# pettni/smooth_feedback

Hardware: AMD Instinct MI355X
Metric: QP solves/sec (higher is better)
Workload: dtype f64

## Files before the change

### smooth_feedback_amd/csrc/qp_sparse.hip

```cpp
#include <hip/hip_runtime.h>

#include <cstdlib>
#include <map>
#include <mutex>

#include <algorithm>
#include <type_traits>
#include <utility>
#include <cfloat>
#include <cmath>

#include "knobs.h"
#include "../../include/sfb.h"
#include "qp_sparse_kernel.h"
#include "wave_util.h"

#ifndef SFB_SWEEP_ASM
#define SFB_SWEEP_ASM 1
#endif
#ifndef SFB_SWEEP_DEPTH
#define SFB_SWEEP_DEPTH 8
#endif

namespace sfb {
// ... 990 lines not shown
                                              vdouble2 (&lx)[8], vint2 (&ix)[8], const bool pre, const bool next, const bool resident = false,
                                              const int treg = 0, const unsigned long long tail_have = 0)
{
  const int k = uni(pl.k);
  const int fu = uni(pl.funits) - treg;
  if (resident) sweep_dev<8, true, false, false, true, kLatResident>(pl.fidx, fu, w.LxF, t, lane, pl.fmask, 0, 0, lx, ix, pl.bidx, w.LxB, pl.bmask);
  else if (pre) sweep_dev<8, true, false, true, true>(pl.fidx, fu, w.LxF, t, lane, pl.fmask, 0, 0, lx, ix, pl.bidx, w.LxB, pl.bmask);
  else sweep_dev<8, true, false, false, true>(pl.fidx, fu, w.LxF, t, lane, pl.fmask, 0, 0, lx, ix, pl.bidx, w.LxB, pl.bmask);
  if constexpr (kLatTail > 0) {
    if (treg > 0) {
      double *const tl = t + (k - 1 - kLatTail) + lane;
      const bool mine = lane >= kLatTail - treg && lane <= kLatTail;
      double tr = mine ? *tl : 0.0;
      auto for_steps = [&]<int... S>(std::integer_sequence<int, S...>, auto &&fn) { (fn(std::integral_constant<int, S>{}), ...); };
      auto block = [&]<int B>(std::integral_constant<int, B>) {
        if (8 * B + 8 > kLatTail - treg) {
          for_steps(std::make_integer_sequence<int, 8>{}, [&]<int E>(std::integral_constant<int, E>) {
            constexpr int S = 8 * B + E;
            int l0, h0;
            asm volatile("v_accvgpr_read_b32 %0, a[%2] ; lat tail (check_sweep_spills.py)\n\tv_accvgpr_read_b32 %1, a[%3]"
                         : "=v"(l0), "=v"(h0)
                         : "n"(kLatTailReg0 + 2 * S), "n"(kLatTailReg0 + 2 * S + 1));
            const double piv = __hiloint2double(__builtin_amdgcn_readlane(__double2hiint(tr), S), __builtin_amdgcn_readlane(__double2loint(tr), S));
            if ((tail_have >> S) & 1) tr = fma(-__hiloint2double(h0, l0), piv, tr);
          });
        }
      };
      for_steps(std::make_integer_sequence<int, kLatTail / 8>{}, block);
      if (mine && lane > kLatTail - treg) *tl = tr;
      wave_lds_fence();
    }
  }
  for (int j0 = lane; j0 < k; j0 += kWave * 8) {
    double dv[8];
#pragma unroll
    for (int e = 0; e < 8; ++e) dv[e] = (j0 + e * kWave < k) ? Dinv[j0 + e * kWave] : 0.0;
#pragma unroll
    for (int e = 0; e < 8; ++e)
      if (j0 + e * kWave < k) t[j0 + e * kWave] = dv[e] * t[j0 + e * kWave];
  }
  wave_lds_fence();
  if (next) sweep_dev<8, true, false, true, true>(pl.bidx, uni(pl.bunits), w.LxB, t, lane, pl.bmask, 0, 0, lx, ix, pl.fidx, w.LxF, pl.fmask);
  else sweep_dev<8, true, false, true, false>(pl.bidx, uni(pl.bunits), w.LxB, t, lane, pl.bmask, 0, 0, lx, ix);
}

template<int UB>
__device__ __forceinline__ double lane_max_abs_b(const double *v, const int len, const int lane)
{
  double r = 0.0;
  for (int e0 = lane; e0 < len; e0 += kWave * UB) {
    double x[UB];
#pragma unroll
    for (int e = 0; e < UB; ++e) x[e] = (e0 + e * kWave < len) ? v[e0 + e * kWave] : 0.0;
#pragma unroll
    for (int e = 0; e < UB; ++e) r = fmax(r, fabs(x[e]));
  }
  return wave_max(r);
}
__device__ __forceinline__ double lane_max_abs(const double *v, int len, int lane)
{
  double r = 0.0;
  for (int e = lane; e < len; e += kWave) r = fmax(r, fabs(v[e]));
  return wave_max(r);
}

constexpr int kRowChunk = 8;
template<class PosF, class IdxF>
__device__ __forceinline__ double sp_row_dot(const int p0, const int p1, const double *vals, PosF pos, IdxF idx,
                                             const double *v)
{
  double s = 0.0;
  for (int q = p0; q < p1; q += kRowChunk) {
    int ps[kRowChunk], ix[kRowChunk];
    double a[kRowChunk], x[kRowChunk];
#pragma unroll
    for (int e = 0; e < kRowChunk; ++e) {
      const bool on = q + e < p1;
      ps[e] = on ? pos(q + e) : 0;
      ix[e] = on ? idx(q + e) : 0;
    }
#pragma unroll
    for (int e = 0; e < kRowChunk; ++e) {
      a[e] = vals[ps[e]];
      x[e] = v[ix[e]];
    }
#pragma unroll
    for (int e = 0; e < kRowChunk; ++e)
      if (q + e < p1) s = fma(a[e], x[e], s);
  }
  return s;
}
template<int RB, int CE, class PtrF, class PosF, class IdxF>
__device__ __forceinline__ void sp_rows_dot(double (&s)[RB], const int i0, const int nrows, PtrF ptr, const double *vals, PosF pos,
                                            IdxF idx, const double *v)
{
  int p[RB], pe[RB];
#pragma unroll
  for (int r = 0; r < RB; ++r) {
    const int i = i0 + r * kWave;
    const bool on = i < nrows;
    p[r]  = on ? ptr(i) : 0;
    pe[r] = on ? ptr(i + 1) : 0;
    s[r]  = 0.0;
  }
  for (;;) {
    bool more = false;
#pragma unroll
    for (int r = 0; r < RB; ++r) more = more || p[r] < pe[r];
    if (!more) break;
    int ps[RB][CE], ix[RB][CE];
    double a[RB][CE], x[RB][CE];
#pragma unroll
    for (int r = 0; r < RB; ++r)
#pragma unroll
      for (int e = 0; e < CE; ++e) {
        const bool on = p[r] + e < pe[r];
        ps[r][e] = on ? pos(p[r] + e) : 0;
        ix[r][e] = on ? idx(p[r] + e) : 0;
      }
#pragma unroll
    for (int r = 0; r < RB; ++r)
#pragma unroll
      for (int e = 0; e < CE; ++e) {
        a[r][e] = vals[ps[r][e]];
        x[r][e] = v[ix[r][e]];
      }
#pragma unroll
    for (int r = 0; r < RB; ++r) {
#pragma unroll
      for (int e = 0; e < CE; ++e)
        if (p[r] + e < pe[r]) s[r] = fma(a[r][e], x[r][e], s[r]);
      p[r] += CE;
    }
  }
}
template<int RB, int CE>
__device__ __forceinline__ void sp_rows_A(double (&s)[RB], const SparsePlanDev &pl, const Item &it, int i0, const double *v)
{
  sp_rows_dot<RB, CE>(s, i0, uni(pl.m), [&](int i) { return pl.Ap[i]; }, it.Ax, [](int p) { return p; },
                      [&](int p) { return pl.Aj[p]; }, v);
}
template<int RB, int CE>
__device__ __forceinline__ void sp_rows_P(double (&s)[RB], const SparsePlanDev &pl, const Item &it, int i0, const double *v)
{
  sp_rows_dot<RB, CE>(s, i0, uni(pl.n), [&](int i) { return pl.Prp[i]; }, it.Px, [&](int p) { return pl.Prpos[p]; },
                      [&](int p) { return pl.Prj[p]; }, v);
}
template<int RB, int CE>
__device__ __forceinline__ void sp_rows_At(double (&s)[RB], const SparsePlanDev &pl, const Item &it, int j0, const double *v)
{
  sp_rows_dot<RB, CE>(s, j0, uni(pl.n), [&](int j) { return pl.Acp[j]; }, it.Ax, [&](int p) { return pl.Acpos[p]; },
                      [&](int p) { return pl.Aci[p]; }, v);
}
__device__ __forceinline__ double sp_row_A(const SparsePlanDev &pl, const Item &it, int i, const double *v)
{
  return sp_row_dot(pl.Ap[i], pl.Ap[i + 1], it.Ax, [](int p) { return p; }, [&](int p) { return pl.Aj[p]; }, v);
}
__device__ __forceinline__ double sp_row_At(const SparsePlanDev &pl, const Item &it, int j, const double *v)
{
  return sp_row_dot(pl.Acp[j], pl.Acp[j + 1], it.Ax, [&](int p) { return pl.Acpos[p]; },
                    [&](int p) { return pl.Aci[p]; }, v);
}
__device__ __forceinline__ double sp_row_P(const SparsePlanDev &pl, const Item &it, int i, const double *v)
{
  return sp_row_dot(pl.Prp[i], pl.Prp[i + 1], it.Px, [&](int p) { return pl.Prpos[p]; },
                    [&](int p) { return pl.Prj[p]; }, v);
}

#ifdef SFB_CHECK_FULL_PASSES
constexpr bool kCheckExit = false;
#else
constexpr bool kCheckExit = true;
#endif
#ifdef SFB_PROF_CHECK
enum { kCkChecks, kCkOptimal, kCkDualRes, kCkOrdered, kCkPass2, kCkPinf, kCkPass3, kCkQdx, kCkRows, kCkDinf, kCkCycOpt, kCkCycCert, kCkCycPass2,
       kCkCycPass3, kCkCycTail, kCkHist2 = 16, kCkHist3 = 32, kCkSlots = 48 };
__device__ unsigned long long sfb_check_prof[2][kCkSlots];
constexpr int kStdWavesPerSimd = 2;
#define SFB_CK_ADD(slot, v) { if (lane == 0) atomicAdd(&sfb_check_prof[RBX > 4][slot], (unsigned long long)(v)); }
#define SFB_CK_LAP(slot) { const unsigned now_ = (unsigned)__builtin_amdgcn_s_memtime(); SFB_CK_ADD(slot, now_ - ck_pc) ck_pc = now_; }
#define SFB_CK_ROW(found, hit, base, j0) { if (!found && wave_ballot(hit)) { found = true; SFB_CK_ADD(base + min((j0) / kWave, 14), 1) } }
#define SFB_CK_HIST(base, found) { if (!found) SFB_CK_ADD(base + 15, 1) }
#else
constexpr int kStdWavesPerSimd = 3;
#define SFB_CK_ADD(slot, v)
#define SFB_CK_LAP(slot)
#define SFB_CK_ROW(found, hit, base, j0)
#define SFB_CK_HIST(base, found)
#endif

template<int RBX = 4>
__device__ inline int sp_check_stopping(const SparsePlanDev &pl, const Item &it, const Ws &w,
                                        const DenseKernelParams &kp, double *t, const int lane, float *score = nullptr)
{
  const int n = uni(pl.n), m = uni(pl.m);
  const double inf = INFINITY;
#ifdef SFB_PROF_CHECK
  unsigned ck_pc = (unsigned)__builtin_amdgcn_s_memtime();
  bool ck_first2 = false, ck_first3 = false;
#endif
  SFB_CK_ADD(kCkChecks, 1)
  const int chunk  = (uni(pl.k) + 1) / 2;
  const double *const xl = t, *const yl = t + n;
  {
    double a = 0.0, r = 0.0, z = 0.0;
    constexpr int RB = RBX, CE = 2;
    for (int i0 = lane; i0 < m; i0 += kWave * RB) {
      double Ax[RB], zi[RB];
#pragma unroll
      for (int rr = 0; rr < RB; ++rr) zi[rr] = (i0 + rr * kWave < m) ? w.zus[i0 + rr * kWave] : 0.0;
      sp_rows_A<RB, CE>(Ax, pl, it, i0, xl);
#pragma unroll
      for (int rr = 0; rr < RB; ++rr) {
        a = fmax(a, fabs(Ax[rr]));
        r = fmax(r, fabs(Ax[rr] - zi[rr]));
        z = fmax(z, fabs(zi[rr]));
      }
    }
    const double Ax_norm = wave_max(a), r_norm = wave_max(r), z_norm = wave_max(z);
    if (score != nullptr && lane == 0) *score = (float)(r_norm / (kp.eps_abs + kp.eps_rel * fmax(Ax_norm, z_norm)));
    if (r_norm <= kp.eps_abs + kp.eps_rel * fmax(Ax_norm, z_norm)) {
      SFB_CK_ADD(kCkDualRes, 1)
      double pn = 0.0, qn = 0.0, an = 0.0, rn = 0.0;
      if constexpr (RBX <= 4) {
      for (int j = lane; j < n; j += kWave) {
        const double Px = sp_row_P(pl, it, j, xl), Aty = sp_row_At(pl, it, j, yl), qj = it.q[j];
        pn = fmax(pn, fabs(Px));
        qn = fmax(qn, fabs(qj));
        an = fmax(an, fabs(Aty));
        rn = fmax(rn, fabs(Px + (qj + Aty)));
      }
      } else
      for (int j0 = lane; j0 < n; j0 += kWave * RB) {
        double Px[RB], Aty[RB], qj[RB];
#pragma unroll
        for (int rr = 0; rr < RB; ++rr) qj[rr] = (j0 + rr * kWave < n) ? it.q[j0 + rr * kWave] : 0.0;
        sp_rows_P<RB, CE>(Px, pl, it, j0, xl);
        sp_rows_At<RB, CE>(Aty, pl, it, j0, yl);
#pragma unroll
        for (int rr = 0; rr < RB; ++rr) {
          pn = fmax(pn, fabs(Px[rr]));
          qn = fmax(qn, fabs(qj[rr]));
          an = fmax(an, fabs(Aty[rr]));
          rn = fmax(rn, fabs(Px[rr] + (qj[rr] + Aty[rr])));
        }
      }
      const double dual_scale = fmax(fmax(wave_max(pn), wave_max(qn)), wave_max(an)), rn_norm = wave_max(rn);
      if (rn_norm <= kp.eps_abs + kp.eps_rel * dual_scale) {
        SFB_CK_ADD(kCkOptimal, 1)
        SFB_CK_LAP(kCkCycOpt)
        return SFB_QP_OPTIMAL;
      }
      if (score != nullptr && lane == 0) *score = (float)(rn_norm / (kp.eps_abs + kp.eps_rel * dual_scale));
    }
  }
  SFB_CK_LAP(kCkCycOpt)
  {
    constexpr int UBV     = RBX > 4 ? 6 : 1;
    const double Edy_norm = lane_max_abs_b<UBV>(w.dyus, m, lane);
    const double thr      = kp.eps_pinf * Edy_norm;
    int side = 2;
    {
      double ps = 0.0, pa = 0.0;
      bool brk0 = false;
      for (int i0 = lane; i0 < m; i0 += kWave * UBV) {
        double uv[UBV], lv[UBV], dv[UBV];
#pragma unroll
        for (int e = 0; e < UBV; ++e) {
          const int i   = i0 + e * kWave;
          const bool on = i < m;
          uv[e] = on ? it.u[i] : 0.0;
          lv[e] = on ? it.l[i] : 0.0;
          dv[e] = on ? w.dyus[i] : 0.0;
        }
#pragma unroll
        for (int e = 0; e < UBV; ++e) {
          if (i0 + e * kWave < m) {
            const double ui = uv[e], li = lv[e], dyi = dv[e];
            const double ta = (ui != inf) ? ui * fmax(0.0, dyi) : 0.0, tb = (li != -inf) ? li * fmin(0.0, dyi) : 0.0;
            ps += ta;
            ps += tb;
            pa += fabs(ta);
            pa += fabs(tb);
            brk0 = brk0 || (ui == inf && dyi > thr) || (li == -inf && dyi < -thr);
          }
        }
      }
      const double sum = wave_sum(ps), S = wave_sum(pa);
      const double err = 4.0 * (2.0 * (double)m) * DBL_EPSILON * S;
      if (!wave_ballot(brk0) && S < inf) {
        if (sum - err >= thr) side = 0;
        else if (sum + err < thr) side = 1;
      }
    }
    double acc = 0.0;
    bool brk   = false;
    if (side == 2) {
    SFB_CK_ADD(kCkOrdered, 1)
    for (int c0 = 0; c0 < m; c0 += chunk) {
      const int c1 = min(m, c0 + chunk);
      for (int i = c0 + lane; i < c1; i += kWave) {
        const double ui = it.u[i], li = it.l[i], dyi = w.dyus[i];
        t[2 * (i - c0)]     = (ui != inf) ? ui * fmax(0.0, dyi) : 0.0;
        t[2 * (i - c0) + 1] = (li != -inf) ? li * fmin(0.0, dyi) : 0.0;
        brk = brk || (ui == inf && dyi > thr) || (li == -inf && dyi < -thr);
      }
      wave_sync();
      {
        const int cnt = 2 * (c1 - c0);
        int e = 0;
        for (; e + 16 <= cnt; e += 16) {
          vdouble2 v[8];
#pragma unroll
          for (int qq = 0; qq < 8; ++qq) v[qq] = *reinterpret_cast<const vdouble2 *>(t + e + 2 * qq);
#pragma unroll
          for (int qq = 0; qq < 8; ++qq) {
            acc += v[qq].x;
            acc += v[qq].y;
          }
        }
        for (; e < cnt; ++e) acc += t[e];
      }
      wave_sync();
    }
    if (wave_ballot(brk)) acc = inf;
    }
    SFB_CK_LAP(kCkCycCert)
    if (side == 1 || (side == 2 && !(acc >= thr))) {
      SFB_CK_ADD(kCkPass2, 1)
      for (int e = lane; e < m; e += kWave) t[e] = w.dyus[e];
      wave_sync();
      double an = 0.0;
      bool open;
      {
        const double r = fabs(lane < n ? sp_row_At(pl, it, lane, t) : 0.0);
        an             = fmax(an, r);
        SFB_CK_ROW(ck_first2, r >= thr, kCkHist2, 0)
        open = !(kCheckExit && wave_ballot(r >= thr));
      }
      if constexpr (RBX <= 4) {
        for (int jb = kWave; open && jb < n; jb += kWave) {
          const int j    = jb + lane;
          const double r = fabs(j < n ? sp_row_At(pl, it, j, t) : 0.0);
          an             = fmax(an, r);
          SFB_CK_ROW(ck_first2, r >= thr, kCkHist2, jb)
          open = !(kCheckExit && wave_ballot(r >= thr));
        }
      } else
      for (int jb = kWave; open && jb < n; jb += kWave * RBX) {
        double Atdy[RBX];
        sp_rows_At<RBX, 2>(Atdy, pl, it, jb + lane, t);
        bool hit = false;
#pragma unroll
        for (int rr = 0; rr < RBX; ++rr) {
          an  = fmax(an, fabs(Atdy[rr]));
          hit = hit || fabs(Atdy[rr]) >= thr;
          SFB_CK_ROW(ck_first2, fabs(Atdy[rr]) >= thr, kCkHist2, jb + rr * kWave)
        }
        open = !(kCheckExit && wave_ballot(hit));
      }
      SFB_CK_HIST(kCkHist2, ck_first2)
      const double Aty_norm = wave_max(an);
      wave_sync();
      const double mxv      = (side == 1 || !(Aty_norm < acc)) ? Aty_norm : acc;
      SFB_CK_LAP(kCkCycPass2)
      if (mxv < thr) {
        SFB_CK_ADD(kCkPinf, 1)
        return SFB_QP_PRIMAL_INFEASIBLE;
      }
    }
  }
  {
    double dmx = 0.0;
    constexpr int UBV = RBX > 4 ? 6 : 1;
    for (int e0 = lane; e0 < n; e0 += kWave * UBV) {
      double v[UBV];
#pragma unroll
      for (int e = 0; e < UBV; ++e) v[e] = (e0 + e * kWave < n) ? w.dxus[e0 + e * kWave] : 0.0;
#pragma unroll
      for (int e = 0; e < UBV; ++e)
        if (e0 + e * kWave < n) {
          t[e0 + e * kWave] = v[e];
          dmx               = fmax(dmx, fabs(v[e]));
        }
    }
    const double dx_norm = wave_max(dmx);
    const double thr     = kp.eps_dinf * dx_norm;
    wave_sync();
    SFB_CK_LAP(kCkCycTail)
    SFB_CK_ADD(kCkPass3, 1)
    double pn = 0.0;
    bool open;
    {
      const double r = fabs(lane < n ? sp_row_P(pl, it, lane, t) : 0.0);
      pn             = fmax(pn, r);
      SFB_CK_ROW(ck_first3, r > thr, kCkHist3, 0)
      open = !(kCheckExit && wave_ballot(r > thr));
    }
    for (int jb = kWave; open && jb < n; jb += kWave * 8) {
      double Pdx[8];
      sp_rows_P<8, 1>(Pdx, pl, it, jb + lane, t);
      bool hit = false;
#pragma unroll
      for (int rr = 0; rr < 8; ++rr) {
        pn  = fmax(pn, fabs(Pdx[rr]));
        hit = hit || fabs(Pdx[rr]) > thr;
        SFB_CK_ROW(ck_first3, fabs(Pdx[rr]) > thr, kCkHist3, jb + rr * kWave)
      }
      open = !(kCheckExit && wave_ballot(hit));
    }
    SFB_CK_HIST(kCkHist3, ck_first3)
    const double Pdx_n = wave_max(pn);
    SFB_CK_LAP(kCkCycPass3)
    if (!(Pdx_n <= thr)) return -1;
    SFB_CK_ADD(kCkQdx, 1)
    wave_sync();
    double qdx = 0.0;
    for (int c0 = 0; c0 < n; c0 += chunk) {
      const int c1 = min(n, c0 + chunk);
      for (int j = c0 + lane; j < c1; j += kWave) {
        t[2 * (j - c0)]     = it.q[j];
        t[2 * (j - c0) + 1] = w.dxus[j];
      }
      wave_sync();
      {
        const int cnt = c1 - c0;
        int e = 0;
        for (; e + 8 <= cnt; e += 8) {
          vdouble2 v[8];
#pragma unroll
          for (int qq = 0; qq < 8; ++qq) v[qq] = *reinterpret_cast<const vdouble2 *>(t + 2 * (e + qq));
#pragma unroll
          for (int qq = 0; qq < 8; ++qq) qdx = fma(v[qq].x, v[qq].y, qdx);
        }
        for (; e < cnt; ++e) qdx = fma(t[2 * e], t[2 * e + 1], qdx);
      }
      wave_sync();
    }
    if (!(qdx <= thr)) {
      SFB_CK_LAP(kCkCycTail)
      return -1;
    }
    SFB_CK_ADD(kCkRows, 1)
    bool rowok = true;
    for (int i = lane; i < m; i += kWave) {
      const double Adx = sp_row_A(pl, it, i, w.dxus), ui = it.u[i], li = it.l[i];
      if (ui == inf) rowok = rowok && (Adx >= -thr);
      else if (li == -inf) rowok = rowok && (Adx <= thr);
      else rowok = rowok && (fabs(Adx) < thr);
    }
    SFB_CK_LAP(kCkCycTail)
    if (!wave_ballot(!rowok)) {
      SFB_CK_ADD(kCkDinf, 1)
      return SFB_QP_DUAL_INFEASIBLE;
    }
  }
  return -1;
}

__device__ __noinline__ void sp_trace_row(const SparsePlanDev &pl, const Item &it, const Ws &w, double *t, const int lane,
                                          const uint32_t iter, const unsigned long long t0_ticks, double *row)
{
  const int n = uni(pl.n), m = uni(pl.m);
  const int chunk = (uni(pl.k) + 1) / 2;
  double pri = 0.0, dua = 0.0, o = 0.0;
  for (int i = lane; i < m; i += kWave) pri = fmax(pri, fabs(sp_row_A(pl, it, i, w.xus) - w.zus[i]));
  for (int c0 = 0; c0 < n; c0 += chunk) {
    const int c1 = min(n, c0 + chunk);
    for (int j = c0 + lane; j < c1; j += kWave) {
      const double Px = sp_row_P(pl, it, j, w.xus), qj = it.q[j];
      dua = fmax(dua, fabs(Px + qj + sp_row_At(pl, it, j, w.yus)));
      t[2 * (j - c0)]     = 0.5 * Px + qj;
      t[2 * (j - c0) + 1] = w.xus[j];
    }
    wave_sync();
    for (int e = 0; e < c1 - c0; ++e) o += t[2 * e] * t[2 * e + 1];
    wave_sync();
  }
  pri = wave_max(pri);
  dua = wave_max(dua);
  if (lane == 0) {
    row[0] = (double)iter;
    row[1] = o;
    row[2] = pri;
    row[3] = dua;
    row[4] = (double)(wall_clock64() - t0_ticks) * 0.01;
  }
}

template<int RB, int CE, class PtrF, class IdxF, class LoadF, class FmaF>
__device__ __forceinline__ void sp_rows_chain(double (&acc)[RB], const int i0, const int nrows, PtrF ptr, IdxF idx, LoadF load, FmaF fm)
{
  using IdxT = decltype(idx(0));
  using ValT = decltype(load(idx(0)));
  int p[RB], pe[RB];
#pragma unroll
  for (int r = 0; r < RB; ++r) {
    const int i = i0 + r * kWave;
    p[r] = pe[r] = 0;
    if (i < nrows) {
      const auto pp = ptr(i);
      p[r]  = pp.a;
      pe[r] = pp.b;
    }
  }
  IdxT ix[RB][CE];
  auto fetch = [&] {
#pragma unroll
    for (int r = 0; r < RB; ++r)
#pragma unroll
      for (int e = 0; e < CE; ++e) ix[r][e] = idx((p[r] + e < pe[r]) ? p[r] + e : 0);
  };
  fetch();
  for (;;) {
    bool more = false;
#pragma unroll
    for (int r = 0; r < RB; ++r) more = more || p[r] < pe[r];
    if (!more) break;
    ValT v[RB][CE];
    IdxT ic[RB][CE];
    bool on[RB][CE];
#pragma unroll
    for (int r = 0; r < RB; ++r)
#pragma unroll
      for (int e = 0; e < CE; ++e) {
        ic[r][e] = ix[r][e];
        v[r][e]  = load(ic[r][e]);
        on[r][e] = p[r] + e < pe[r];
      }
#pragma unroll
    for (int r = 0; r < RB; ++r) p[r] += CE;
    fetch();
#pragma unroll
    for (int r = 0; r < RB; ++r)
#pragma unroll
      for (int e = 0; e < CE; ++e)
        if (on[r][e]) acc[r] = fm(r, ic[r][e], v[r][e], acc[r]);
  }
}

template<int SD, bool WIDE = false>
__device__ inline void sp_polish(const SparsePlanDev &pl, const Item &it, const Ws &w, const Ws &wf, const DenseKernelParams &kp,
                                 double *t, const double c, const int lane, const bool lean)
{
  const int n = uni(pl.n), m = uni(pl.m), k = uni(pl.k);
  const double inf = INFINITY, eps = DBL_EPSILON;
  for (int i = lane; i < m; i += kWave) {
    const double yi = w.ys[i];
    double a        = 0.0;
    if (yi < -100 * eps && it.l[i] != -inf) a = 1.0;
    if (yi > 100 * eps && it.u[i] != inf) a = 2.0;
    w.act[i] = a;
  }
  for (int e = lane; e < k; e += kWave) w.tv[e] = 0.0;
// ... 384 lines not shown
#pragma unroll
        for (int a = 0; a < kRowChunk; ++a) xv[a] = wx[j[a]];
#pragma unroll
        for (int a = 0; a < kRowChunk; ++a)
          if (q + a < q1) acc = fma(syi * av[a], xv[a], acc);
      }
      w.zs[i] = acc;
    }
  } else {
    for (int j = lane; j < n; j += kWave) w.xs[j] = 0.0;
    for (int i = lane; i < m; i += kWave) {
      w.ys[i] = 0.0;
      w.zs[i] = 0.0;
    }
  }
  wave_sync();
  }

  if (ph1 == PH_SETUP) {
    if (lane == 0) {
      w.hdr[0] = c;
      w.hdr[1] = 0.0;
      w.hdr[2] = (double)next_chk;
      w.hdr[3] = (double)t0_ticks;
#ifdef SFB_SP_TIMELINE
      w.hdr[4] = (double)tl0;
      w.hdr[5] = (double)tl1;
#endif
      w.hdr[kHdrCode]     = (double)ret_code;
      w.hdr[kHdrComplete] = 0.0;
    }
    return SP_DONE;
  }

  const uint32_t iter0 = iter;
  bool need_rhs        = true;
  double *vxs = w.xs, *vqc = w.qc, *vys = w.ys, *vzs = w.zs, *vrinv = w.rinv, *vrho = w.rho, *vlo = w.lo, *vhi = w.hi;
  const int32_t *vpinv = pl.pinv;
  [[maybe_unused]] double *vdinv = nullptr;
  [[maybe_unused]] const uint16_t *vp16 = nullptr;
  [[maybe_unused]] const uint8_t *vcls  = nullptr;
  const double rho_c0 = 1e-6, rho_c1 = 1e3 * kp.rho_bar, rho_c2 = kp.rho_bar;
  const double rinv_c0 = 1.0 / rho_c0, rinv_c1 = 1.0 / rho_c1, rinv_c2 = 1.0 / rho_c2;
  auto pinv_at = [&](const int e) -> int {
    if constexpr (LAT) return (int)vp16[e];
    else return vpinv[e];
  };
  auto rho_at = [&](const int i) -> double {
    if constexpr (LAT) { const int cl = vcls[i]; return cl == 0 ? rho_c0 : (cl == 1 ? rho_c1 : rho_c2); }
    else return vrho[i];
  };
  auto rinv_at = [&](const int i) -> double {
    if constexpr (LAT) { const int cl = vcls[i]; return cl == 0 ? rinv_c0 : (cl == 1 ? rinv_c1 : rinv_c2); }
    else return vrinv[i];
  };
  const bool iterates  = ph0 <= PH_ADMM && iter != maxit && ret_code < 0;
  constexpr int kLatRows = kLatRegRows;
  if constexpr (LAT) {
    if (n > kLatRows * kWave || m > kLatRows * kWave) __builtin_trap();
  }
  [[maybe_unused]] double xr[kLatRows], yr[kLatRows], zr[kLatRows];
  [[maybe_unused]] double *lqc = nullptr, *llo = nullptr, *lhi = nullptr;
  [[maybe_unused]] const double *lrtab = nullptr;
  auto regs_to_lds = [&](const double (&v)[kLatRows], double *dst, const int len) {
    double *const dl = dst + lane;
#pragma unroll
    for (int r = 0; r < kLatRows; ++r)
      if (lane < len - r * kWave) dl[r * kWave] = v[r];
  };
  auto lds_to_regs = [&](double (&v)[kLatRows], const double *src, const int len) {
    const double *const sl = src + lane;
#pragma unroll
    for (int r = 0; r < kLatRows; ++r) v[r] = (lane < len - r * kWave) ? sl[r * kWave] : 0.0;
  };
  [[maybe_unused]] auto copy_in = [&](double *dst, const double *src, const int len) {
    constexpr int UB = 6;
    for (int e0 = lane; e0 < len; e0 += kWave * UB) {
      double v[UB];
#pragma unroll
      for (int e = 0; e < UB; ++e) v[e] = (e0 + e * kWave < len) ? src[e0 + e * kWave] : 0.0;
#pragma unroll
      for (int e = 0; e < UB; ++e)
        if (e0 + e * kWave < len) dst[e0 + e * kWave] = v[e];
    }
  };
  auto iterate_in = [&] {
    if constexpr (LAT) {
      copy_in(t, w.xs, n);
      copy_in(t + n, w.ys, m);
      copy_in(lhi, w.zs, m);
      wave_sync();
      lds_to_regs(xr, t, n);
      lds_to_regs(yr, t + n, m);
      lds_to_regs(zr, lhi, m);
      wave_sync();
      copy_in(lhi, w.hi, m);
      wave_sync();
    }
  };
  if constexpr (LAT) {
    double *cq = t + ((k + 2) & ~1), *clo = cq + n, *chi = clo + m;
    lqc = cq; llo = clo; lhi = chi;
    vdinv = chi + m;
    constexpr int kPad = kLatRows * kWave;
    double *ltab = vdinv + k;
    lrtab = ltab;
    uint16_t *lp = reinterpret_cast<uint16_t *>(ltab + 8);
    uint8_t *lc  = reinterpret_cast<uint8_t *>(lp + 2 * kPad);
    vp16 = lp;
    vcls = lc;
#pragma unroll
    for (int r = 0; r < kLatRows; ++r) xr[r] = yr[r] = zr[r] = 0.0;
    if (iterates) {
      copy_in(cq, w.qc, n);
      copy_in(clo, w.lo, m);
#pragma unroll 1
      for (int e0 = lane; e0 < kPad; e0 += 4 * kWave) {
        int px[4], py[4];
        double rho[4];
#pragma unroll
        for (int q = 0; q < 4; ++q) {
          const int e = e0 + q * kWave;
          px[q]  = e < n ? pl.pinv[e] : k;
          py[q]  = e < m ? pl.pinv[n + e] : k;
          rho[q] = e < m ? w.rho[e] : rho_c2;
        }
#pragma unroll
        for (int q = 0; q < 4; ++q) {
          const int e  = e0 + q * kWave;
          lp[e]        = (uint16_t)(8 * px[q]);
          lp[kPad + e] = (uint16_t)(8 * py[q]);
          lc[e]        = (uint8_t)(8 * (rho[q] == rho_c0 ? 0 : (rho[q] == rho_c1 ? 1 : 2)));
        }
      }
      if (lane < 3) {
        ltab[lane]     = lane == 0 ? rinv_c0 : (lane == 1 ? rinv_c1 : rinv_c2);
        ltab[3 + lane] = lane == 0 ? rho_c0 : (lane == 1 ? rho_c1 : rho_c2);
      }
      copy_in(vdinv, w.Dinv, k);
      iterate_in();
    }
  }
  [[maybe_unused]] bool lat_resident = false;
  [[maybe_unused]] int lat_treg = 0;
  [[maybe_unused]] unsigned long long lat_have = 0;
  if constexpr (LAT) {
    if (iterates && uni(pl.funits) >= 8 && uni(pl.bunits) >= 8) lat_treg = lat_tail_units(pl);
    lat_resident = iterates && uni(pl.idx_scale) == 8 && uni(pl.bunits) >= 8 && lat_resident_ok(pl, lat_treg);
    if (lat_resident) lat_resident_load(w.LxF, lane);
    if constexpr (kLatTail > 0) {
      if (lat_treg > 0) lat_have = lat_tail_load(pl, w.LxF, lane, lat_treg);
    }
  }
  auto vectors_home = [&] {
    if constexpr (LAT) {
      if (iterates) {
        wave_sync();
        regs_to_lds(xr, t, n);
        regs_to_lds(yr, t + n, m);
        regs_to_lds(zr, lhi, m);
        wave_sync();
        for (int j = lane; j < n; j += kWave) w.xs[j] = t[j];
        for (int i = lane; i < m; i += kWave) { w.ys[i] = t[n + i]; w.zs[i] = lhi[i]; }
        wave_sync();
      }
    }
  };
#if defined(SFB_ITER_EXP) && SFB_ITER_EXP >= 3
  if constexpr (LAT) { vqc = vxs; vlo = vys; vhi = vzs; }
#endif
  [[maybe_unused]] const bool lat_chain = LAT && uni(pl.idx_scale) == 8 && uni(pl.funits) >= 8 && uni(pl.bunits) >= 8;
  for (; ph0 <= PH_ADMM && iter != maxit && ret_code < 0; ++iter) {
    constexpr int UNR_A = LAT ? 8 : 4, UNR_B = 4;
    [[maybe_unused]] auto t_at = [&](const int off) -> double & { return *reinterpret_cast<double *>(reinterpret_cast<char *>(t) + off); };
    [[maybe_unused]] double v_alpha = kp.alpha, v_alphac = kp.alpha_comp, v_sigma = kp.sigma;
    if constexpr (LAT) asm volatile("" : "+v"(v_alpha), "+v"(v_alphac), "+v"(v_sigma));
    [[maybe_unused]] auto tab_at = [&](const int off) -> double { return *reinterpret_cast<const double *>(reinterpret_cast<const char *>(lrtab) + off); };
    [[maybe_unused]] auto rhs_from_regs = [&] {
      constexpr int kPad = kLatRows * kWave;
      int pv[kLatRows];
      double qv[kLatRows];
#pragma unroll
      for (int r = 0; r < kLatRows; ++r) {
        pv[r] = (int)vp16[lane + r * kWave];
        qv[r] = lqc[lane + r * kWave];
      }
#pragma unroll
      for (int r = 0; r < kLatRows; ++r) t_at(pv[r]) = v_sigma * xr[r] - qv[r];
#pragma unroll
      for (int r = 0; r < kLatRows; ++r) {
        pv[r] = (int)vp16[kPad + lane + r * kWave];
        qv[r] = tab_at((int)vcls[lane + r * kWave]);
      }
#pragma unroll
      for (int r = 0; r < kLatRows; ++r) t_at(pv[r]) = zr[r] - qv[r] * yr[r];
    };
    if constexpr (LAT) {
      if (iter == next_chk) {
        wave_sync();
        regs_to_lds(xr, t, n);
        regs_to_lds(yr, t + n, m);
        wave_sync();
        for (int j = lane; j < n; j += kWave) w.dxus[j] = t[j];
        for (int i = lane; i < m; i += kWave) w.dyus[i] = t[n + i];
        wave_sync();
        need_rhs = true;
      }
      if (need_rhs) rhs_from_regs();
    } else
    if (need_rhs) {
    constexpr int UNR = UNR_A;
    for (int j0 = lane; j0 < n; j0 += kWave * UNR) {
      double xv[UNR], qv[UNR];
      int pv[UNR];
#pragma unroll
      for (int e = 0; e < UNR; ++e) {
        const int j = j0 + e * kWave;
        const bool on = j < n;
        xv[e] = on ? vxs[j] : 0.0;
        qv[e] = on ? vqc[j] : 0.0;
        pv[e] = on ? pinv_at(j) : k;
      }
#pragma unroll
      for (int e = 0; e < UNR; ++e)
        if (j0 + e * kWave < n) t[pv[e]] = kp.sigma * xv[e] - qv[e];
    }
    for (int i0 = lane; i0 < m; i0 += kWave * UNR) {
      double zv[UNR], rv[UNR], yv[UNR];
      int pv[UNR];
#pragma unroll
      for (int e = 0; e < UNR; ++e) {
        const int i = i0 + e * kWave;
        const bool on = i < m;
        zv[e] = on ? vzs[i] : 0.0;
        rv[e] = on ? rinv_at(i) : 0.0;
        yv[e] = on ? vys[i] : 0.0;
        pv[e] = on ? pinv_at(n + i) : k;
      }
#pragma unroll
      for (int e = 0; e < UNR; ++e)
        if (i0 + e * kWave < m) t[pv[e]] = zv[e] - rv[e] * yv[e];
    }
    }
    const bool chk = (iter == next_chk);
    wave_sync();
#if defined(SFB_ITER_EXP) && SFB_ITER_EXP == 2
    if (false)
#endif
    if constexpr (LAT) {
      if (lat_chain && !lean) {
        vdouble2 lat_lx[8];
        vint2 lat_ix[8];
        ldl_solve_lat(pl, w, t, lane, vdinv, lat_lx, lat_ix, false, false, lat_resident, lat_treg, lat_have);
      } else {
        ldl_solve_dev<8>(pl, w, t, lane, lean, vdinv);
      }
    } else {
      ldl_solve_dev<SFB_SWEEP_DEPTH>(pl, w, t, lane, lean, nullptr);
    }
    if (chk) next_chk += sci;
    need_rhs = chk;
    if constexpr (!LAT) {
      if (chk) {
        for (int j = lane; j < n; j += kWave) w.dxus[j] = vxs[j];
        for (int i = lane; i < m; i += kWave) w.dyus[i] = vys[i];
      }
    }
    auto xrows = [&]<int U, bool PRED>(std::integral_constant<int, U>, std::bool_constant<PRED>, const int r0) {
      double xo[U], qv[U];
      int pv[U];
#pragma unroll
      for (int e = 0; e < U; ++e) {
        const int j   = lane + (r0 + e) * kWave;
        const bool on = !PRED || j < n;
        xo[e] = on ? vxs[j] : 0.0;
        qv[e] = on ? vqc[j] : 0.0;
        pv[e] = on ? pinv_at(j) : k;
      }
#pragma unroll
      for (int e = 0; e < U; ++e) {
        const int j = lane + (r0 + e) * kWave;
        if (!PRED || j < n) {
          const double xn = kp.alpha * t[pv[e]] + kp.alpha_comp * xo[e];
          vxs[j]   = xn;
          t[pv[e]] = kp.sigma * xn - qv[e];
        }
      }
    };
    auto yrows = [&]<int U, bool PRED>(std::integral_constant<int, U>, std::bool_constant<PRED>, const int r0) {
      double yo[U], zo[U], ri[U], rh[U], lo[U], hi[U];
      int pv[U];
#pragma unroll
      for (int e = 0; e < U; ++e) {
        const int i   = lane + (r0 + e) * kWave;
        const bool on = !PRED || i < m;
        yo[e] = on ? vys[i] : 0.0;
        zo[e] = on ? vzs[i] : 0.0;
        ri[e] = on ? rinv_at(i) : 0.0;
        rh[e] = on ? rho_at(i) : 0.0;
        lo[e] = on ? vlo[i] : 0.0;
        hi[e] = on ? vhi[i] : 0.0;
        pv[e] = on ? pinv_at(n + i) : k;
      }
#pragma unroll
      for (int e = 0; e < U; ++e) {
        const int i = lane + (r0 + e) * kWave;
        if (!PRED || i < m) {
          const double nu = t[pv[e]];
          double zn = kp.alpha * (ri[e] * nu) + kp.alpha_comp * (ri[e] * yo[e]) + zo[e];
          zn = (zn < lo[e]) ? lo[e] : zn;
          zn = (hi[e] < zn) ? hi[e] : zn;
          const double yn = kp.alpha_comp * yo[e] + kp.alpha * nu + rh[e] * zo[e] - rh[e] * zn;
          vys[i]   = yn;
          vzs[i]   = zn;
          t[pv[e]] = zn - ri[e] * yn;
        }
      }
    };
    auto all_rows = [&]<int U>(std::integral_constant<int, U> uu, const int len, auto &&rows) {
      const int full = len / kWave;
      int r = 0;
      for (; r + U <= full; r += U) rows(uu, std::false_type{}, r);
      if constexpr (U > 4) if (r + 4 <= full) { rows(std::integral_constant<int, 4>{}, std::false_type{}, r); r += 4; }
      if constexpr (U > 2) if (r + 2 <= full) { rows(std::integral_constant<int, 2>{}, std::false_type{}, r); r += 2; }
      if constexpr (U > 1) if (r + 1 <= full) { rows(std::integral_constant<int, 1>{}, std::false_type{}, r); r += 1; }
      if (full * kWave < len) rows(std::integral_constant<int, 1>{}, std::true_type{}, r);
    };
#if defined(SFB_ITER_EXP) && SFB_ITER_EXP == 1
    if (false)
#endif
    if constexpr (LAT) {
      constexpr int kPad = kLatRows * kWave;
      auto xbatch = [&]<int R0, int RN>(std::integral_constant<int, R0>, std::integral_constant<int, RN>) {
        if (R0 * kWave >= n) return;
        int pv[RN];
        double qv[RN], tv[RN];
#pragma unroll
        for (int e = 0; e < RN; ++e) {
          pv[e] = (int)vp16[lane + (R0 + e) * kWave];
          qv[e] = lqc[lane + (R0 + e) * kWave];
        }
#pragma unroll
        for (int e = 0; e < RN; ++e) tv[e] = t_at(pv[e]);
#pragma unroll
        for (int e = 0; e < RN; ++e) {
          const double xn = v_alpha * tv[e] + v_alphac * xr[R0 + e];
          xr[R0 + e]  = xn;
          t_at(pv[e]) = v_sigma * xn - qv[e];
        }
      };
      auto ybatch = [&]<int R0, int RN>(std::integral_constant<int, R0>, std::integral_constant<int, RN>) {
        if (R0 * kWave >= m) return;
        int pv[RN], cl[RN];
        double lo[RN], hi[RN], tv[RN], riv[RN], rhv[RN];
#pragma unroll
        for (int e = 0; e < RN; ++e) {
          const int i = lane + (R0 + e) * kWave;
          pv[e] = (int)vp16[kPad + i];
          cl[e] = (int)vcls[i];
          lo[e] = llo[i];
          hi[e] = lhi[i];
        }
#pragma unroll
        for (int e = 0; e < RN; ++e) {
          tv[e]  = t_at(pv[e]);
          riv[e] = tab_at(cl[e]);
          rhv[e] = tab_at(cl[e] + 24);
        }
#pragma unroll
        for (int e = 0; e < RN; ++e) {
          const double ri = riv[e], rh = rhv[e];
          const double nu = tv[e], yo = yr[R0 + e], zo = zr[R0 + e];
          double zn = v_alpha * (ri * nu) + v_alphac * (ri * yo) + zo;
          zn = (zn < lo[e]) ? lo[e] : zn;
          zn = (hi[e] < zn) ? hi[e] : zn;
          const double yn = v_alphac * yo + v_alpha * nu + rh * zo - rh * zn;
          yr[R0 + e]  = yn;
          zr[R0 + e]  = zn;
          t_at(pv[e]) = zn - ri * yn;
        }
      };
      static_assert(kLatRows == 12, "batches of the register form");
      xbatch(std::integral_constant<int, 0>{}, std::integral_constant<int, 6>{});
      xbatch(std::integral_constant<int, 6>{}, std::integral_constant<int, 6>{});
      ybatch(std::integral_constant<int, 0>{}, std::integral_constant<int, 4>{});
      ybatch(std::integral_constant<int, 4>{}, std::integral_constant<int, 4>{});
      ybatch(std::integral_constant<int, 8>{}, std::integral_constant<int, 4>{});
    } else
    {
    all_rows(std::integral_constant<int, UNR_A>{}, n, xrows);
    all_rows(std::integral_constant<int, UNR_B>{}, m, yrows);
    }
    if constexpr (LAT) {
      if (chk) {
        vectors_home();
        vxs = t; vys = t + n; vzs = lhi;
      }
    }
    if (chk) {
      constexpr int UBU = LAT ? 6 : 1;
      for (int j0 = lane; j0 < n; j0 += kWave * UBU) {
        double sxv[UBU], xov[UBU];
#pragma unroll
        for (int e = 0; e < UBU; ++e) {
          const bool on = j0 + e * kWave < n;
          sxv[e] = on ? w.sx[j0 + e * kWave] : 0.0;
          xov[e] = on ? w.dxus[j0 + e * kWave] : 0.0;
        }
#pragma unroll
        for (int e = 0; e < UBU; ++e) {
          const int j = j0 + e * kWave;
          if (j < n) {
            const double xn = vxs[j], sxj = sxv[e], xo = xov[e];
            w.xus[j]  = sxj * xn;
            t[j]      = sxj * xn;
            w.dxus[j] = sxj * (xn - xo);
          }
        }
      }
      for (int i0 = lane; i0 < m; i0 += kWave * UBU) {
        double syv[UBU], yov[UBU];
#pragma unroll
        for (int e = 0; e < UBU; ++e) {
          const bool on = i0 + e * kWave < m;
          syv[e] = on ? w.sy[i0 + e * kWave] : 1.0;
          yov[e] = on ? w.dyus[i0 + e * kWave] : 0.0;
        }
#pragma unroll
        for (int e = 0; e < UBU; ++e) {
          const int i = i0 + e * kWave;
          if (i < m) {
            const double yn = vys[i], zn = vzs[i], syi = syv[e], yo = yov[e];
            w.yus[i]  = syi * yn / c;
            t[n + i]  = syi * yn / c;
            w.zus[i]  = (1.0 / syi) * zn;
            w.dyus[i] = syi * (yn - yo) / c;
          }
        }
      }
    }
    wave_sync();
    if (chk) {
      ret_code = sp_check_stopping<LAT ? 6 : 4>(pl, it, w, kp, t, lane, pause_at != 0 ? score : nullptr);
      if constexpr (TRACE) {
        if (trace != nullptr && trace_rows < trace_cap) sp_trace_row(pl, it, w, t, lane, iter, t0_ticks, trace + ((size_t)b * (size_t)trace_cap + (size_t)trace_rows) * 5);
        ++trace_rows;
      }
      if (ret_code < 0 && max_time_exceeded(kp.max_time_ns, t0_ticks)) ret_code = SFB_QP_MAX_TIME;
      wave_sync();
      if constexpr (LAT) iterate_in();
      lean = __builtin_amdgcn_readfirstlane(__hip_atomic_load(pl.dev_active, __ATOMIC_RELAXED, __HIP_MEMORY_SCOPE_AGENT)) >
             lean_waves;
      if (iter > 600) __builtin_amdgcn_s_setprio(3);
      else if (iter > 300) __builtin_amdgcn_s_setprio(2);
      else if (iter > 100) __builtin_amdgcn_s_setprio(1);
      if (pause_at != 0 && ret_code < 0 && iter + 1 >= pause_at && iter + 1 != maxit) {
        if (lane == 0) {
          w.hdr[0] = c;
          w.hdr[1] = (double)(iter + 1);
          w.hdr[2] = (double)next_chk;
          w.hdr[3] = (double)t0_ticks;
#ifdef SFB_SP_TIMELINE
          w.hdr[4] = (double)tl0;
          w.hdr[5] = (double)tl1;
#endif
          w.hdr[kHdrCode]     = -1.0;
          w.hdr[kHdrComplete] = 0.0;
        }
        __builtin_amdgcn_s_setprio(0);
        vectors_home();
        return SP_PAUSED;
      }
      if (queue != nullptr && ret_code < 0 && iter + 1 != maxit && iter + 1 - iter0 >= slice) {
        int wait = 0;
        if (lane == 0) {
          const int fresh = __hip_atomic_load(&queue[kQFresh], __ATOMIC_RELAXED, __HIP_MEMORY_SCOPE_AGENT);
          const int head  = __hip_atomic_load(&queue[kQHead], __ATOMIC_RELAXED, __HIP_MEMORY_SCOPE_AGENT);
          const int tail  = __hip_atomic_load(&queue[kQTail], __ATOMIC_RELAXED, __HIP_MEMORY_SCOPE_AGENT);
          wait            = (fresh < batch) || (tail - head > 0);
        }
        if (__builtin_amdgcn_readfirstlane(wait)) {
          if (lane == 0) {
            w.hdr[0] = c;
            w.hdr[1] = (double)(iter + 1);
            w.hdr[2] = (double)next_chk;
            w.hdr[3] = (double)t0_ticks;
#ifdef SFB_SP_TIMELINE
            w.hdr[4] = (double)tl0;
            w.hdr[5] = (double)tl1;
#endif
          }
          __builtin_amdgcn_s_setprio(0);
          vectors_home();
          return SP_SUSPENDED;
        }
      }
    }
  }
  __builtin_amdgcn_s_setprio(0);
  vectors_home();

#ifdef SFB_SP_TIMELINE
  tl2 = wall_clock64();
#endif
  if (ph1 == PH_ADMM) {
    if (lane == 0) {
      w.hdr[0] = c;
      w.hdr[1] = (double)iter;
      w.hdr[kHdrCode] = (double)ret_code;
#ifdef SFB_SP_TIMELINE
      w.hdr[kHdrTl2] = (double)tl2;
#endif
    }
    return SP_DONE;
  }
#ifdef SFB_SP_TIMELINE
  if (ph0 == PH_FINISH) tl2 = (unsigned long long)w.hdr[kHdrTl2];
#endif
  phase_lap(3);
  if (ret_code == SFB_QP_OPTIMAL && kp.polish) {
    if (kp.reuse != 0 && allow_reuse) {
      const Ws wp = polish_ws(w, gws + slot * ws_doubles,
                              qp_sparse_polish_offset(n, m, uni(pl.nnzL), uni(pl.funits), uni(pl.bunits), pl.Aorig ? nnzA : 0), n, m,
                              uni(pl.nnzL), uni(pl.funits), uni(pl.bunits));
      sp_polish<SFB_SWEEP_DEPTH, WIDE>(pl, it, w, wp, kp, t, c, lane, lean);
    } else {
      if (lane == 0) w.hdr[kHdrStamp] = 0.0;
      sp_polish<SFB_SWEEP_DEPTH, WIDE>(pl, it, w, w, kp, t, c, lane, lean);
    }
  }

  phase_lap(4);
  double *ox = gx + b * (size_t)n, *oy = gy + b * (size_t)m;
  for (int j = lane; j < n; j += kWave) {
    const double v = w.sx[j] * w.xs[j];
    ox[j]    = v;
    w.xus[j] = v;
  }
  for (int i = lane; i < m; i += kWave) oy[i] = w.sy[i] * w.ys[i] / c;
  wave_sync();
  if (gobj != nullptr) {
    const int chunk = (k + 1) / 2;
    double o        = 0.0;
    for (int c0 = 0; c0 < n; c0 += chunk) {
      const int c1 = min(n, c0 + chunk);
      struct Ix { int a, b; };
      struct V2 { double a, b; };
      constexpr int RB = 4, CE = 2;
      for (int i0 = c0 + lane; i0 < c1; i0 += kWave * RB) {
        double acc[RB], xi[RB], qi[RB];
#pragma unroll
        for (int r = 0; r < RB; ++r) {
          const int i = i0 + r * kWave;
          acc[r] = 0.0;
          xi[r]  = (i < c1) ? w.xus[i] : 0.0;
          qi[r]  = (i < c1) ? it.q[i] : 0.0;
        }
        sp_rows_chain<RB, CE>(acc, i0, c1, [&](int i) { return Ix{pl.Prp[i], pl.Prp[i + 1]}; },
                              [&](int q) { return Ix{pl.Prpos[q], pl.Prj[q]}; },
                              [&](const Ix &x) { return V2{it.Px[x.a], w.xus[x.b]}; },
                              [&](int, const Ix &, const V2 &v, double a) { return fma(0.5 * v.a, v.b, a); });
#pragma unroll
        for (int r = 0; r < RB; ++r) {
          const int i = i0 + r * kWave;
          if (i < c1) {
            t[2 * (i - c0)]     = xi[r];
            t[2 * (i - c0) + 1] = acc[r] + qi[r];
          }
        }
      }
      wave_sync();
      const int cnt = c1 - c0;
      int e = 0;
      for (; e + 8 <= cnt; e += 8) {
        vdouble2 v[8];
#pragma unroll
        for (int qq = 0; qq < 8; ++qq) v[qq] = *reinterpret_cast<const vdouble2 *>(t + 2 * (e + qq));
#pragma unroll
        for (int qq = 0; qq < 8; ++qq) o = fma(v[qq].x, v[qq].y, o);
      }
      for (; e < cnt; ++e) o = fma(t[2 * e], t[2 * e + 1], o);
      wave_sync();
    }
    if (lane == 0) gobj[b] = o;
  }
  if (lane == 0) {
    gcode[b] = (ret_code >= 0) ? ret_code : SFB_QP_MAX_ITERATIONS;
    if (giter != nullptr) giter[b] = iter;
#ifdef SFB_SP_TIMELINE
    oy[0] = (double)tl0; oy[1] = (double)tl1; oy[2] = (double)tl2; oy[3] = (double)wall_clock64();
#endif
  }
  if constexpr (TRACE) {
    wave_sync();
    phase_lap(5);
    if (phase_us != nullptr && lane == 0)
      for (int i = 0; i < 6; ++i) phase_us[b * 6 + i] = (double)ph_t[i] * 0.01;
  }
  return SP_DONE;
}

}

// ... 561 lines not shown
```

Measured before the change: 233,600.

## Stage check-step vectors in LDS and use wide register-row A products in LAT checks

In the latency (LAT) path, the convergence check now keeps the scaled dual and primal deltas and z in LDS buffers (llo, lqc, t) instead of re-reading them from global workspace. It adds a wide sparse A-row product that processes all register rows per lane with 3-element chunks. Full wave barriers are replaced with LDS fences at check points, and after the check the iterate is restored with a cheaper iterate_back that reloads x/y and bounds directly. The aim is to cut global-memory traffic and synchronisation in the periodic termination check. The cost is extra LDS buffer reuse (lqc, llo, lhi are overwritten and must be reloaded afterwards), which adds correctness risk.

```diff
diff --git a/smooth_feedback_amd/csrc/qp_sparse.hip b/smooth_feedback_amd/csrc/qp_sparse.hip
--- a/smooth_feedback_amd/csrc/qp_sparse.hip
+++ b/smooth_feedback_amd/csrc/qp_sparse.hip
@@ -1166,6 +1166,78 @@
   sp_rows_dot<RB, CE>(s, j0, uni(pl.n), [&](int j) { return pl.Acp[j]; }, it.Ax, [&](int p) { return pl.Acpos[p]; },
                       [&](int p) { return pl.Aci[p]; }, v);
 }
+template<int RB, int CE>
+__device__ __forceinline__ void sp_rows_A_wide(double (&s)[RB], const SparsePlanDev &pl, const Item &it, const int lane, const double *v)
+{
+  const int m = uni(pl.m);
+  int p[RB], pe[RB];
+  {
+    const int32_t *const ap = pl.Ap + lane;
+#pragma unroll
+    for (int r = 0; r < RB; ++r) {
+      const bool on = lane < m - r * kWave;
+      p[r]  = on ? ap[r * kWave] : 0;
+      pe[r] = on ? ap[r * kWave + 1] : 0;
+      s[r]  = 0.0;
+    }
+  }
+  for (;;) {
+    bool more = false;
+#pragma unroll
+    for (int r = 0; r < RB; ++r) more = more || p[r] + CE <= pe[r];
+    if (!more) break;
+    int ix[RB][CE];
+    double a[RB][CE];
+#pragma unroll
+    for (int r = 0; r < RB; ++r) {
+      const int b0             = (p[r] + CE <= pe[r]) ? p[r] : 0;
+      const int32_t *const jp = pl.Aj + b0;
+      const double *const xp  = it.Ax + b0;
+#pragma unroll
+      for (int e = 0; e < CE; ++e) {
+        ix[r][e] = jp[e];
+        a[r][e]  = xp[e];
+      }
+    }
+    __builtin_amdgcn_sched_barrier(0);
+#pragma unroll
+    for (int r = 0; r < RB; ++r) {
+      const bool on = p[r] + CE <= pe[r];
+      double x[CE], sr = s[r];
+#pragma unroll
+      for (int e = 0; e < CE; ++e) x[e] = v[ix[r][e]];
+#pragma unroll
+      for (int e = 0; e < CE; ++e) sr = fma(a[r][e], x[e], sr);
+      s[r] = on ? sr : s[r];
+      p[r] += on ? CE : 0;
+    }
+  }
+  bool rest = false;
+#pragma unroll
+  for (int r = 0; r < RB; ++r) rest = rest || p[r] < pe[r];
+  if (rest) {
+    int ix[RB][CE - 1];
+    double a[RB][CE - 1];
+#pragma unroll
+    for (int r = 0; r < RB; ++r)
+#pragma unroll
+      for (int e = 0; e < CE - 1; ++e) {
+        const int q = (p[r] + e < pe[r]) ? p[r] + e : 0;
+        ix[r][e]    = pl.Aj[q];
+        a[r][e]     = it.Ax[q];
+      }
+    __builtin_amdgcn_sched_barrier(0);
+#pragma unroll
+    for (int r = 0; r < RB; ++r) {
+      double x[CE - 1];
+#pragma unroll
+      for (int e = 0; e < CE - 1; ++e) x[e] = v[ix[r][e]];
+#pragma unroll
+      for (int e = 0; e < CE - 1; ++e)
+        if (p[r] + e < pe[r]) s[r] = fma(a[r][e], x[e], s[r]);
+    }
+  }
+}
 __device__ __forceinline__ double sp_row_A(const SparsePlanDev &pl, const Item &it, int i, const double *v)
 {
   return sp_row_dot(pl.Ap[i], pl.Ap[i + 1], it.Ax, [](int p) { return p; }, [&](int p) { return pl.Aj[p]; }, v);
@@ -1203,10 +1275,15 @@
 #define SFB_CK_HIST(base, found)
 #endif
 
+constexpr int kProbeCE = 16;
 template<int RBX = 4>
 __device__ inline int sp_check_stopping(const SparsePlanDev &pl, const Item &it, const Ws &w,
-                                        const DenseKernelParams &kp, double *t, const int lane, float *score = nullptr)
-{
+                                        const DenseKernelParams &kp, double *t, const int lane, float *score = nullptr,
+                                        [[maybe_unused]] const double *dyl = nullptr, [[maybe_unused]] const double *dxl = nullptr)
+{
+  constexpr bool WIDE = RBX > 4;
+  int ol = lane;
+  if constexpr (WIDE) asm volatile("" : "+v"(ol));
   const int n = uni(pl.n), m = uni(pl.m);
   const double inf = INFINITY;
 #ifdef SFB_PROF_CHECK
@@ -1219,6 +1296,19 @@
   {
     double a = 0.0, r = 0.0, z = 0.0;
     constexpr int RB = RBX, CE = 2;
+    if constexpr (WIDE) {
+      double Ax[kLatRegRows], zi[kLatRegRows];
+      sp_rows_A_wide<kLatRegRows, 3>(Ax, pl, it, ol, xl);
+      const double *const zl = t + n + ol;
+#pragma unroll
+      for (int rr = 0; rr < kLatRegRows; ++rr) zi[rr] = (ol < m - rr * kWave) ? zl[rr * kWave] : 0.0;
+#pragma unroll
+      for (int rr = 0; rr < kLatRegRows; ++rr) {
+        a = fmax(a, fabs(Ax[rr]));
+        r = fmax(r, fabs(Ax[rr] - zi[rr]));
+        z = fmax(z, fabs(zi[rr]));
+      }
+    } else
     for (int i0 = lane; i0 < m; i0 += kWave * RB) {
       double Ax[RB], zi[RB];
 #pragma unroll
@@ -1236,6 +1326,18 @@
     if (r_norm <= kp.eps_abs + kp.eps_rel * fmax(Ax_norm, z_norm)) {
       SFB_CK_ADD(kCkDualRes, 1)
       double pn = 0.0, qn = 0.0, an = 0.0, rn = 0.0;
+      if constexpr (WIDE) {
+        wave_sync();
+        double yv[kLatRegRows];
+        const double *const ys = w.yus + ol;
+        double *const yd       = t + n + ol;
+#pragma unroll
+        for (int rr = 0; rr < kLatRegRows; ++rr) yv[rr] = (ol < m - rr * kWave) ? ys[rr * kWave] : 0.0;
+#pragma unroll
+        for (int rr = 0; rr < kLatRegRows; ++rr)
+          if (ol < m - rr * kWave) yd[rr * kWave] = yv[rr];
+        wave_sync();
+      }
       if constexpr (RBX <= 4) {
       for (int j = lane; j < n; j += kWave) {
         const double Px = sp_row_P(pl, it, j, xl), Aty = sp_row_At(pl, it, j, yl), qj = it.q[j];
@@ -1270,14 +1372,15 @@
   }
   SFB_CK_LAP(kCkCycOpt)
   {
-    constexpr int UBV     = RBX > 4 ? 6 : 1;
-    const double Edy_norm = lane_max_abs_b<UBV>(w.dyus, m, lane);
+    constexpr int UBV     = WIDE ? kLatRegRows : 1;
+    const double *const dyv = WIDE ? dyl : w.dyus;
+    const double Edy_norm = lane_max_abs_b<UBV>(dyv, m, ol);
     const double thr      = kp.eps_pinf * Edy_norm;
     int side = 2;
     {
       double ps = 0.0, pa = 0.0;
       bool brk0 = false;
-      for (int i0 = lane; i0 < m; i0 += kWave * UBV) {
+      for (int i0 = ol; i0 < m; i0 += kWave * UBV) {
         double uv[UBV], lv[UBV], dv[UBV];
 #pragma unroll
         for (int e = 0; e < UBV; ++e) {
@@ -1285,7 +1388,7 @@
           const bool on = i < m;
           uv[e] = on ? it.u[i] : 0.0;
           lv[e] = on ? it.l[i] : 0.0;
-          dv[e] = on ? w.dyus[i] : 0.0;
+          dv[e] = on ? dyv[i] : 0.0;
         }
 #pragma unroll
         for (int e = 0; e < UBV; ++e) {
@@ -1314,7 +1417,7 @@
     for (int c0 = 0; c0 < m; c0 += chunk) {
       const int c1 = min(m, c0 + chunk);
       for (int i = c0 + lane; i < c1; i += kWave) {
-        const double ui = it.u[i], li = it.l[i], dyi = w.dyus[i];
+        const double ui = it.u[i], li = it.l[i], dyi = dyv[i];
         t[2 * (i - c0)]     = (ui != inf) ? ui * fmax(0.0, dyi) : 0.0;
         t[2 * (i - c0) + 1] = (li != -inf) ? li * fmin(0.0, dyi) : 0.0;
         brk = brk || (ui == inf && dyi > thr) || (li == -inf && dyi < -thr);
@@ -1342,12 +1445,21 @@
     SFB_CK_LAP(kCkCycCert)
     if (side == 1 || (side == 2 && !(acc >= thr))) {
       SFB_CK_ADD(kCkPass2, 1)
+      const double *dyg = t;
+      if constexpr (WIDE) dyg = dyl;
+      else {
       for (int e = lane; e < m; e += kWave) t[e] = w.dyus[e];
       wave_sync();
+      }
       double an = 0.0;
       bool open;
       {
-        const double r = fabs(lane < n ? sp_row_At(pl, it, lane, t) : 0.0);
+        double r;
+        if constexpr (WIDE) {
+          double pr[1];
+          sp_rows_At<1, kProbeCE>(pr, pl, it, ol, dyg);
+          r = fabs(pr[0]);
+        } else r = fabs(lane < n ? sp_row_At(pl, it, lane, t) : 0.0);
         an             = fmax(an, r);
         SFB_CK_ROW(ck_first2, r >= thr, kCkHist2, 0)
         open = !(kCheckExit && wave_ballot(r >= thr));
@@ -1363,7 +1475,7 @@
       } else
       for (int jb = kWave; open && jb < n; jb += kWave * RBX) {
         double Atdy[RBX];
-        sp_rows_At<RBX, 2>(Atdy, pl, it, jb + lane, t);
+        sp_rows_At<RBX, 2>(Atdy, pl, it, jb + lane, dyg);
         bool hit = false;
 #pragma unroll
         for (int rr = 0; rr < RBX; ++rr) {
@@ -1386,7 +1498,12 @@
   }
   {
     double dmx = 0.0;
-    constexpr int UBV = RBX > 4 ? 6 : 1;
+    constexpr int UBV = 1;
+    const double *dxg = t;
+    if constexpr (WIDE) {
+      dxg = dxl;
+      dmx = lane_max_abs_b<kLatRegRows>(dxl, n, ol);
+    } else
     for (int e0 = lane; e0 < n; e0 += kWave * UBV) {
       double v[UBV];
 #pragma unroll
@@ -1406,14 +1523,19 @@
     double pn = 0.0;
     bool open;
     {
-      const double r = fabs(lane < n ? sp_row_P(pl, it, lane, t) : 0.0);
+      double r;
+      if constexpr (WIDE) {
+        double pr[1];
+        sp_rows_P<1, kProbeCE>(pr, pl, it, ol, dxg);
+        r = fabs(pr[0]);
+      } else r = fabs(lane < n ? sp_row_P(pl, it, lane, t) : 0.0);
       pn             = fmax(pn, r);
       SFB_CK_ROW(ck_first3, r > thr, kCkHist3, 0)
       open = !(kCheckExit && wave_ballot(r > thr));
     }
     for (int jb = kWave; open && jb < n; jb += kWave * 8) {
       double Pdx[8];
-      sp_rows_P<8, 1>(Pdx, pl, it, jb + lane, t);
+      sp_rows_P<8, 1>(Pdx, pl, it, jb + lane, dxg);
       bool hit = false;
 #pragma unroll
       for (int rr = 0; rr < 8; ++rr) {
@@ -2104,18 +2226,41 @@
       if (lat_treg > 0) lat_have = lat_tail_load(pl, w.LxF, lane, lat_treg);
     }
   }
-  auto vectors_home = [&] {
+  auto vectors_home = [&](const bool at_check = false) {
     if constexpr (LAT) {
       if (iterates) {
-        wave_sync();
+        if (at_check) wave_lds_fence(); else wave_sync();
         regs_to_lds(xr, t, n);
         regs_to_lds(yr, t + n, m);
         regs_to_lds(zr, lhi, m);
-        wave_sync();
+        if (at_check) wave_lds_fence(); else wave_sync();
         for (int j = lane; j < n; j += kWave) w.xs[j] = t[j];
         for (int i = lane; i < m; i += kWave) { w.ys[i] = t[n + i]; w.zs[i] = lhi[i]; }
-        wave_sync();
-      }
+        if (at_check) wave_lds_fence(); else wave_sync();
+      }
+    }
+  };
+  [[maybe_unused]] auto iterate_back = [&] {
+    if constexpr (LAT) {
+      lds_to_regs(zr, lhi, m);
+      wave_lds_fence();
+      int ol = lane;
+      asm volatile("" : "+v"(ol));
+      auto rows_in = [&](double (&v)[kLatRows], const double *src, const int len) {
+        const double *const sl = src + ol;
+#pragma unroll
+        for (int r = 0; r < kLatRows; ++r) v[r] = (ol < len - r * kWave) ? sl[r * kWave] : 0.0;
+      };
+      double bh[kLatRows], bq[kLatRows], bl[kLatRows];
+      rows_in(xr, w.xs, n);
+      rows_in(yr, w.ys, m);
+      rows_in(bh, w.hi, m);
+      rows_in(bq, w.qc, n);
+      rows_in(bl, w.lo, m);
+      regs_to_lds(bh, lhi, m);
+      regs_to_lds(bq, lqc, n);
+      regs_to_lds(bl, llo, m);
+      wave_lds_fence();
     }
   };
 #if defined(SFB_ITER_EXP) && SFB_ITER_EXP >= 3
@@ -2345,13 +2490,15 @@
     }
     if constexpr (LAT) {
       if (chk) {
-        vectors_home();
+        vectors_home(true);
         vxs = t; vys = t + n; vzs = lhi;
       }
     }
     if (chk) {
-      constexpr int UBU = LAT ? 6 : 1;
-      for (int j0 = lane; j0 < n; j0 += kWave * UBU) {
+      constexpr int UBU = LAT ? kLatRows : 1;
+      int ul = lane;
+      if constexpr (LAT) asm volatile("" : "+v"(ul));
+      for (int j0 = ul; j0 < n; j0 += kWave * UBU) {
         double sxv[UBU], xov[UBU];
 #pragma unroll
         for (int e = 0; e < UBU; ++e) {
@@ -2367,10 +2514,11 @@
             w.xus[j]  = sxj * xn;
             t[j]      = sxj * xn;
             w.dxus[j] = sxj * (xn - xo);
+            if constexpr (LAT) lqc[j] = sxj * (xn - xo);
           }
         }
       }
-      for (int i0 = lane; i0 < m; i0 += kWave * UBU) {
+      for (int i0 = ul; i0 < m; i0 += kWave * UBU) {
         double syv[UBU], yov[UBU];
 #pragma unroll
         for (int e = 0; e < UBU; ++e) {
@@ -2384,23 +2532,29 @@
           if (i < m) {
             const double yn = vys[i], zn = vzs[i], syi = syv[e], yo = yov[e];
             w.yus[i]  = syi * yn / c;
-            t[n + i]  = syi * yn / c;
+            if constexpr (!LAT) t[n + i] = syi * yn / c;
             w.zus[i]  = (1.0 / syi) * zn;
             w.dyus[i] = syi * (yn - yo) / c;
+            if constexpr (LAT) {
+              t[n + i] = (1.0 / syi) * zn;
+              llo[i]   = syi * (yn - yo) / c;
+            }
           }
         }
       }
     }
-    wave_sync();
+    if constexpr (LAT) {
+      if (chk) wave_lds_fence(); else wave_sync();
+    } else wave_sync();
     if (chk) {
-      ret_code = sp_check_stopping<LAT ? 6 : 4>(pl, it, w, kp, t, lane, pause_at != 0 ? score : nullptr);
+      ret_code = sp_check_stopping<LAT ? 6 : 4>(pl, it, w, kp, t, lane, pause_at != 0 ? score : nullptr, LAT ? llo : nullptr, LAT ? lqc : nullptr);
       if constexpr (TRACE) {
         if (trace != nullptr && trace_rows < trace_cap) sp_trace_row(pl, it, w, t, lane, iter, t0_ticks, trace + ((size_t)b * (size_t)trace_cap + (size_t)trace_rows) * 5);
         ++trace_rows;
       }
       if (ret_code < 0 && max_time_exceeded(kp.max_time_ns, t0_ticks)) ret_code = SFB_QP_MAX_TIME;
       wave_sync();
-      if constexpr (LAT) iterate_in();
+      if constexpr (LAT) iterate_back();
       lean = __builtin_amdgcn_readfirstlane(__hip_atomic_load(pl.dev_active, __ATOMIC_RELAXED, __HIP_MEMORY_SCOPE_AGENT)) >
              lean_waves;
       if (iter > 600) __builtin_amdgcn_s_setprio(3);
```

Result: no change. 235,600, median of 6 (+0.9%).
